# ChenKaiXuSan/Skiing_Analysis_PyTorch

Measured on AMD Instinct MI355X. Metric: 3D-pose frames/sec, 8-view 518px clips, higher is better.
Workload: dtype f16

## Files before the change

### include/skimi.h

```cpp
#ifndef SKIMI_H
#define SKIMI_H

#include <stddef.h>
#include <stdint.h>

#ifdef __cplusplus
extern "C" {
#endif

#define SKIMI_OK 0
#define SKIMI_ERR_ARG (-1)
#define SKIMI_ERR_HIP (-2)
#define SKIMI_ERR_STATE (-3)
#define SKIMI_ERR_WORKSPACE (-4)

#define SKIMI_F32 0
#define SKIMI_BF16 1
#define SKIMI_BF16X3_REC 2
#define SKIMI_FP8MX 3
#define SKIMI_F16 4

#define SKIMI_PREC_BF16 0
#define SKIMI_PREC_BF16X3 1
#define SKIMI_PREC_FP8 2
// ... 59 lines not shown
int skimi_gemm(const skimi_gemm_desc* d, void* stream);

#define SKIMI_GEMM_PATH_GENERIC 1
#define SKIMI_GEMM_PATH_SPLITK_ORDERED 2
#define SKIMI_GEMM_PATH_SPLITK_ATOMIC 3
#define SKIMI_GEMM_PATH_X3DMA_WIDE 4
#define SKIMI_GEMM_PATH_X3DMA_NARROW 5
#define SKIMI_GEMM_PATH_GEMM256 6
#define SKIMI_GEMM_PATH_CONV_WIN 7
int32_t skimi_gemm_last_path(void);

int skimi_quant_mx(const void* x, int32_t dtype, int64_t ldx, int64_t rows, int32_t K, void* payload, void* scales,
                   void* stream);
int skimi_layernorm_mx(const float* x, int64_t ldx, int64_t rows, int32_t C, const float* gamma, const float* beta,
                       float eps, void* payload, void* scales, void* stream);
int skimi_gemm_fp8(const void* A, const void* A_scales, const void* W, const void* W_scales, int32_t M, int32_t N,
                   int32_t K, const float* bias, int32_t act, const float* gamma, const float* resid, int64_t ldr,
                   void* out, int32_t out_dtype, int64_t ldo, void* out_scales, void* stream);

int skimi_conv3x3_n32_pack(const float* w, void* packed, int32_t C, void* stream);
int skimi_conv3x3_n32(const void* in_hi, const void* in_lo, const void* packed_w, const float* bias, float* out,
                      int32_t F, int32_t H, int32_t W, int32_t C, int32_t relu, void* stream);

int skimi_resample_u8(const uint8_t* in, uint8_t* out, int64_t outer, int32_t n_in, int32_t n_out, int64_t inner,
                      const int32_t* kk, const int32_t* bounds, int32_t ksize, void* stream);
int skimi_u8_hwc_to_f32_chw(const uint8_t* in, int32_t H, int32_t W, float* out, int32_t OH, int32_t OW, int32_t y_off,
                            int32_t x_off, float fill, void* stream);

int skimi_layernorm(const float* x, const float* x2, int64_t ldx, int64_t rows, int32_t C,
                    const float* gamma, const float* beta, float eps,
                    void* out, int32_t out_dtype, int64_t ldo, void* stream);

int skimi_qknorm_rope(void* qkv, int32_t dtype, int64_t tokens, int32_t heads,
                      const float* qn_w, const float* qn_b, const float* kn_w, const float* kn_b,
                      float eps, const int32_t* pos, const float* rope_cos, const float* rope_sin,
                      int32_t rope_npos, void* stream);

int skimi_attention(const void* qkv, void* out, int32_t dtype, int32_t batch, int32_t seq,
                    int32_t heads, int32_t head_dim, void* stream);
int skimi_attention_out(const void* qkv, void* out, int32_t dtype, int32_t out_dtype, int32_t batch, int32_t seq,
                        int32_t heads, int32_t head_dim, void* stream);

int skimi_qknorm_rope_scaled(void* qkv, int32_t dtype, int64_t tokens, int32_t heads,
                             const float* qn_w, const float* qn_b, const float* kn_w, const float* kn_b,
                             float eps, const int32_t* pos, const float* rope_cos, const float* rope_sin,
                             int32_t rope_npos, float q_scale, int32_t* q_scaled, void* stream);
// ... 80 lines not shown
```

### skiing_analysis_pytorch_amd/_lib.py

```python
from __future__ import annotations

import ctypes as C
from pathlib import Path

LIB_PATH = Path(__file__).resolve().parent / "lib" / "libskimi.so"

F32, BF16 = 0, 1
F16 = 4
BF16X3_REC = 2
FP8MX = 3
PREC_BF16, PREC_BF16X3, PREC_FP8 = 0, 1, 2
PREC_F16 = 3
ACT_NONE, ACT_RELU, ACT_GELU, ACT_SILU, ACT_SIGMOID = 0, 1, 2, 3, 4
GEMM_PATH_GENERIC, GEMM_PATH_SPLITK_ORDERED, GEMM_PATH_SPLITK_ATOMIC = 1, 2, 3
GEMM_PATH_X3DMA_WIDE, GEMM_PATH_X3DMA_NARROW, GEMM_PATH_GEMM256, GEMM_PATH_CONV_WIN = 4, 5, 6, 7


class SkimiError(RuntimeError):
    pass


class GemmDesc(C.Structure):

    _fields_ = [
# ... 29 lines not shown

_vp = C.c_void_p
_SIGNATURES = {
    "skimi_last_error": (C.c_char_p, []),
    "skimi_version": (C.c_int, []),
    "skimi_sizeof_gemm_desc": (C.c_int, []),
    "skimi_device_count": (C.c_int, []),
    "skimi_profile_start": (C.c_int, [C.c_int32, C.c_int64]),
    "skimi_profile_stop": (C.c_int, [C.POINTER(C.c_double), C.POINTER(C.c_int64), C.POINTER(C.c_double),
                                    C.POINTER(C.c_double)]),
    "skimi_gemm": (C.c_int, [C.POINTER(GemmDesc), _vp]),
    "skimi_gemm_last_path": (C.c_int32, []),
    "skimi_quant_mx": (C.c_int, [_vp, C.c_int32, C.c_int64, C.c_int64, C.c_int32, _vp, _vp, _vp]),
    "skimi_layernorm_mx": (C.c_int, [_vp, C.c_int64, C.c_int64, C.c_int32, _vp, _vp, C.c_float, _vp, _vp, _vp]),
    "skimi_gemm_fp8": (C.c_int, [_vp, _vp, _vp, _vp, C.c_int32, C.c_int32, C.c_int32, _vp, C.c_int32, _vp, _vp, C.c_int64,
                                 _vp, C.c_int32, C.c_int64, _vp, _vp]),
    "skimi_split_planes": (C.c_int, [_vp, C.c_int64, C.c_int64, C.c_int32, _vp, _vp, _vp]),
    "skimi_split_records": (C.c_int, [_vp, C.c_int64, C.c_int64, C.c_int32, _vp, _vp]),
    "skimi_resample_u8": (C.c_int, [_vp, _vp, C.c_int64, C.c_int32, C.c_int32, C.c_int64, _vp, _vp, C.c_int32, _vp]),
    "skimi_u8_hwc_to_f32_chw": (C.c_int, [_vp, C.c_int32, C.c_int32, _vp, C.c_int32, C.c_int32, C.c_int32, C.c_int32,
                                          C.c_float, _vp]),
    "skimi_conv3x3_n32_pack": (C.c_int, [_vp, _vp, C.c_int32, _vp]),
    "skimi_conv3x3_n32": (C.c_int, [_vp, _vp, _vp, _vp, _vp, C.c_int32, C.c_int32, C.c_int32, C.c_int32, C.c_int32, _vp]),
    "skimi_layernorm": (C.c_int, [_vp, _vp, C.c_int64, C.c_int64, C.c_int32, _vp, _vp, C.c_float, _vp,
                                  C.c_int32, C.c_int64, _vp]),
    "skimi_qknorm_rope": (C.c_int, [_vp, C.c_int32, C.c_int64, C.c_int32, _vp, _vp, _vp, _vp, C.c_float,
                                    _vp, _vp, _vp, C.c_int32, _vp]),
    "skimi_attention": (C.c_int, [_vp, _vp, C.c_int32, C.c_int32, C.c_int32, C.c_int32, C.c_int32, _vp]),
    "skimi_attention_out": (C.c_int, [_vp, _vp, C.c_int32, C.c_int32, C.c_int32, C.c_int32, C.c_int32, C.c_int32, _vp]),
    "skimi_qknorm_rope_scaled": (C.c_int, [_vp, C.c_int32, C.c_int64, C.c_int32, _vp, _vp, _vp, _vp, C.c_float,
                                           _vp, _vp, _vp, C.c_int32, C.c_float, C.POINTER(C.c_int32), _vp]),
    "skimi_attention_ex": (C.c_int, [_vp, _vp, C.c_int32, C.c_int32, C.c_int32, C.c_int32, C.c_int32, C.c_int32, C.c_int32,
                                     _vp, C.c_uint64, C.POINTER(C.c_int32), _vp]),
    "skimi_attention_x3_scratch_bytes": (C.c_uint64, [C.c_int64, C.c_int64]),
    "skimi_vp3d_create": (_vp, [C.c_int32, C.c_int32, C.c_int32, C.POINTER(C.c_int32), C.c_int32,
                                C.c_int32, C.c_int32]),
    "skimi_vp3d_destroy": (None, [_vp]),
    "skimi_vp3d_set_weight": (C.c_int, [_vp, C.c_char_p, _vp, C.c_int64]),
    "skimi_vp3d_finalize": (C.c_int, [_vp, C.c_int32]),
    "skimi_vp3d_receptive_field": (C.c_int32, [_vp]),
    "skimi_vp3d_workspace_bytes": (C.c_size_t, [_vp, C.c_int32, C.c_int32]),
    "skimi_vp3d_forward": (C.c_int, [_vp, _vp, _vp, C.c_int32, C.c_int32, _vp, C.c_size_t, _vp]),
    "skimi_pose_to_cameras": (C.c_int, [_vp, C.c_int64, C.c_int32, C.c_int32, _vp, _vp, _vp]),
    "skimi_unproject_depth": (C.c_int, [_vp, _vp, _vp, _vp, C.c_int32, C.c_int32, C.c_int32, _vp]),
    "skimi_triangulate_dlt": (C.c_int, [_vp, _vp, _vp, _vp, _vp, C.c_int64, C.c_int32, C.c_int32, _vp]),
    "skimi_icp_workspace_bytes": (C.c_size_t, [C.c_int64, C.c_int64]),
# ... 67 lines not shown
```

### skiing_analysis_pytorch_amd/csrc/api.hip

```cpp
#include <stdarg.h>

#include <mutex>
#include <vector>

#include "common.h"
#include "gemm_epilogue.h"
#include "kernels.h"

namespace skimi {

static thread_local char g_err[512] = "";

void set_error(const char* fmt, ...) {
    va_list ap;
    va_start(ap, fmt);
    vsnprintf(g_err, sizeof(g_err), fmt, ap);
    va_end(ap);
}

int lds_opt_in(std::atomic<unsigned>& done, const void* kernel, int bytes, const char* what) {
    int dev = 0;
    if (hipGetDevice(&dev) != hipSuccess) {
        set_error("hipGetDevice failed (%s)", what);
        return SKIMI_ERR_HIP;
    }
    const unsigned bit = 1u << (dev & 31);
    if (done.load(std::memory_order_acquire) & bit) return SKIMI_OK;
    const hipError_t e = hipFuncSetAttribute(kernel, hipFuncAttributeMaxDynamicSharedMemorySize, bytes);
    if (e != hipSuccess) {
        set_error("hipFuncSetAttribute(%s, %d bytes of LDS) failed: %s", what, bytes, hipGetErrorString(e));
// ... 96 lines not shown
}

int skimi_resample_u8(const uint8_t* in, uint8_t* out, int64_t outer, int32_t n_in, int32_t n_out, int64_t inner,
                      const int32_t* kk, const int32_t* bounds, int32_t ksize, void* stream) {
    return resample_u8_launch(in, out, outer, n_in, n_out, inner, kk, bounds, ksize, (hipStream_t)stream);
}

int skimi_u8_hwc_to_f32_chw(const uint8_t* in, int32_t H, int32_t W, float* out, int32_t OH, int32_t OW, int32_t y_off,
                            int32_t x_off, float fill, void* stream) {
    return u8_hwc_to_f32_chw_launch(in, H, W, out, OH, OW, y_off, x_off, fill, (hipStream_t)stream);
}

int skimi_conv3x3_n32_pack(const float* w, void* packed, int32_t C, void* stream) {
    SKIMI_CHECK_ARG(w && packed && C > 0, "skimi_conv3x3_n32_pack: bad arguments");
    return conv_direct_pack_launch(w, (unsigned short*)packed, C, (hipStream_t)stream);
}

int skimi_conv3x3_n32(const void* in_hi, const void* in_lo, const void* packed_w, const float* bias, float* out,
                      int32_t F, int32_t H, int32_t W, int32_t C, int32_t relu, void* stream) {
    return conv_direct_n32_launch((const unsigned short*)in_hi, (const unsigned short*)in_lo,
                                  (const unsigned short*)packed_w, bias, out, F, H, W, C, relu, (hipStream_t)stream);
}

int skimi_split_planes(const float* x, int64_t ld, int64_t rows, int32_t C, void* hi, void* lo, void* stream) {
    SKIMI_CHECK_ARG(x && hi && lo && rows > 0 && C > 0, "skimi_split_planes: bad arguments");
    return split_planes_launch(x, (long)ld, (long)rows, C, hi, lo, (hipStream_t)stream);
}

int skimi_split_records(const float* x, int64_t ld, int64_t rows, int32_t C, void* records, void* stream) {
    SKIMI_CHECK_ARG(x && records && rows > 0 && C > 0, "skimi_split_records: bad arguments");
    return split_records_launch(x, (long)ld, (long)rows, C, records, (hipStream_t)stream);
}

int skimi_quant_mx(const void* x, int32_t dtype, int64_t ldx, int64_t rows, int32_t K, void* payload, void* scales,
                   void* stream) {
    return quant_mx_launch(x, dtype, (long)ldx, (long)rows, K, payload, scales, (hipStream_t)stream);
}

int skimi_layernorm_mx(const float* x, int64_t ldx, int64_t rows, int32_t C, const float* gamma, const float* beta,
                       float eps, void* payload, void* scales, void* stream) {
    return layernorm_mx_launch(x, ldx, rows, C, gamma, beta, eps, payload, scales, (hipStream_t)stream);
}

int skimi_gemm_fp8(const void* A, const void* A_scales, const void* W, const void* W_scales, int32_t M, int32_t N,
                   int32_t K, const float* bias, int32_t act, const float* gamma, const float* resid, int64_t ldr,
                   void* out, int32_t out_dtype, int64_t ldo, void* out_scales, void* stream) {
// ... 70 lines not shown
```

### skiing_analysis_pytorch_amd/csrc/conv_direct.hip

```cpp
#include "common.h"
#include "kernels.h"

namespace skimi {

typedef __attribute__((address_space(3))) void lds_void;
typedef __attribute__((address_space(1))) const void gbl_void;

__device__ uint4 g_conv_zero_page[4] = {{0, 0, 0, 0}, {0, 0, 0, 0}, {0, 0, 0, 0}, {0, 0, 0, 0}};

constexpr int CD_WIN = 18 * 18;
constexpr int CD_IN_PLANE = 21 * 1024;
constexpr int CD_W_PLANE = 9 * 32 * 64;
constexpr int CD_BUF = 2 * CD_IN_PLANE + 2 * CD_W_PLANE;

__global__ void conv_direct_pack_kernel(const float* __restrict__ w, unsigned short* __restrict__ out, int Cin) {
    const long n = 32L * Cin * 9;
    for (long i = (long)blockIdx.x * 256 + threadIdx.x; i < n; i += (long)gridDim.x * 256) {
        const int c32 = (int)(i % 32);
        const int co = (int)((i / 32) % 32);
        const int tap = (int)((i / 1024) % 9);
        const int cs = (int)(i / 9216);
        const float v = w[((long)co * Cin + cs * 32 + c32) * 9 + tap];
        const unsigned short hi = f2bf(v);
        const unsigned short lo = f2bf(v - bf2f(hi));
// ... 157 lines not shown
}

int conv_direct_n32_launch(const unsigned short* in_hi, const unsigned short* in_lo, const unsigned short* w_packed,
                           const float* bias, float* out, int F, int H, int W, int C, int relu, hipStream_t st,
                           long px_stride) {
    SKIMI_CHECK_ARG(in_hi && in_lo && w_packed && out, "conv_direct: null buffer");
    SKIMI_CHECK_ARG(C % 32 == 0 && C >= 32 && F > 0 && H > 0 && W > 0, "conv_direct: bad shape");
    SKIMI_CHECK_ARG((((uintptr_t)in_hi | (uintptr_t)in_lo | (uintptr_t)w_packed) & 15) == 0, "conv_direct: 16-B alignment");
    constexpr size_t lds = 2ull * CD_BUF;
    SKIMI_LDS_OPT_IN(conv_direct_n32_kernel, lds, "conv_direct");
    ConvDirectArgs a;
    a.in_hi = in_hi; a.in_lo = in_lo; a.w = w_packed; a.bias = bias; a.out = out;
    a.F = F; a.H = H; a.W = W; a.C = C; a.relu = relu;
    a.px_stride = px_stride > 0 ? px_stride : C;
    a.tiles_x = (int)cdiv(W, 16);
    a.tiles_y = (int)cdiv(H, 16);
    const long nblk = (long)F * a.tiles_x * a.tiles_y;
    SKIMI_CHECK_ARG(nblk < (1l << 31), "conv_direct: grid too large");
    hipLaunchKernelGGL(conv_direct_n32_kernel, dim3((unsigned)nblk), dim3(512), lds, st, a);
    SKIMI_LAUNCH_CHECK();
    return SKIMI_OK;
}

}
```

### skiing_analysis_pytorch_amd/csrc/kernels.h

```cpp
#pragma once
#include "common.h"

namespace skimi {

int gemm_dispatch(const skimi_gemm_desc* d, hipStream_t st, void* scratch, size_t scratch_bytes,
                  int force_splitk);

int layernorm_launch(const float* x, const float* x2, int64_t ldx, int64_t rows, int C,
                     const float* gamma, const float* beta, float eps, void* out, int out_dtype,
                     int64_t ldo, hipStream_t st, int64_t grp_rows = 0, int64_t grp_stride = 0,
                     int64_t grp_off = 0);

int qknorm_rope_launch(void* qkv, int dtype, int64_t tokens, int heads, const float* qn_w,
                       const float* qn_b, const float* kn_w, const float* kn_b, float eps,
                       const int32_t* pos, const float* rope_cos, const float* rope_sin, int rope_npos,
                       hipStream_t st, float q_scale = 1.f, int* q_scaled = nullptr);

struct AttnArgs {
    const void* q;
    const void* k;
    const void* v;
    void* out;
    long q_row, k_row, v_row, o_row;
    long q_batch, k_batch, v_batch, o_batch;
    long q_head, k_head, v_head, o_head;
    int batch, heads, seq_q, seq_k, head_dim;
    float scale;
    int batch_inner = 0;
    long q_batch2 = 0, k_batch2 = 0, v_batch2 = 0, o_batch2 = 0;
    int q_prescaled = 0;
    int out_f16 = 0;
    void* out_mx = nullptr;
    void* out_mx_scales = nullptr;
    long mx_row = 0, mx_srow = 0;
};
bool attention_mx_output_ok(int dtype, int heads, int head_dim);
int attention_f32_launch(const AttnArgs& a, hipStream_t st);
int attention_bf16_launch(const AttnArgs& a, hipStream_t st);
int resample_u8_launch(const unsigned char* in, unsigned char* out, long outer, int n_in, int n_out, long inner,
                       const int* kk, const int* bounds, int ksize, hipStream_t st);
int u8_hwc_to_f32_chw_launch(const unsigned char* in, int H, int W, float* out, int OH, int OW, int y_off, int x_off,
                             float fill, hipStream_t st);
int conv_direct_pack_launch(const float* w, unsigned short* out, int Cin, hipStream_t st);
int conv_direct_n32_launch(const unsigned short* in_hi, const unsigned short* in_lo, const unsigned short* w_packed,
                           const float* bias, float* out, int F, int H, int W, int C, int relu, hipStream_t st,
                           long px_stride = 0);
void attention_q64_dispatch(const AttnArgs& a, hipStream_t st);
int attention_launch(const void* qkv, void* out, int dtype, int batch, int seq, int heads, int head_dim,
                     hipStream_t st, int q_prescaled = 0, void* x3_scratch = nullptr, size_t x3_scratch_bytes = 0,
                     int* out_records = nullptr,
                     int out_f16 = 0,
                     void* out_mx = nullptr, void* out_mx_scales = nullptr);
size_t attention_x3_scratch_bytes(long tokens, long row_elems);
int attention_x3_launch(const AttnArgs& a, long tokens, long row_elems, void* scratch, size_t scratch_bytes, hipStream_t st,
                        bool out_records = false);

int vp3d_im2col_launch(const float* x, float* a0, int B, int L, int Cin, int k, int Kpad, hipStream_t st);

int quant_mx_launch(const void* x, int dtype, long ldx, long rows, int K, void* q, void* scales, hipStream_t st);
int gemm_fp8_launch(const void* A, const void* As, const void* W, const void* Ws, int M, int N, int K, const float* bias, int act,
                    const float* gamma, const float* resid, long ldr, void* out, int out_dtype, long ldo, hipStream_t st,
                    void* out_scales = nullptr);
bool gemm_fp8_mx_output_ok(int M, int N);
int layernorm_mx_launch(const float* x, int64_t ldx, int64_t rows, int C, const float* gamma, const float* beta, float eps,
                        void* payload, void* scales, hipStream_t st);

int vp3d_expand_launch(const float* x, const float* w, int ldw, const float* bias, float* out_f32, void* out_rec, int B, int Lin,
                       int Cin, int taps, int C, hipStream_t st);
int vp3d_expand_mfma_launch(const float* x, const void* wfrag, int Kpad, const float* bias, float* out_f32, void* out_rec, int B,
// ... 7 lines not shown
```

### skiing_analysis_pytorch_amd/csrc/vggt.hip

```cpp
#include <math.h>
#include <string.h>

#include <map>
#include <memory>
#include <string>
#include <tuple>
#include <atomic>
#include <mutex>
#include <vector>

#include <stdlib.h>

#include "common.h"
#include "gemm_epilogue.h"
#include "kernels.h"
#include "track_kernels.h"
#include "vggt_kernels.h"

using namespace skimi;

namespace {

struct Lin {
    void* w = nullptr;
// ... 642 lines not shown
        if (!c.rc && !c.dry()) c.rc = bilinear_ac_launch(olow, o, adt, F, h0, w0, h1, w1, feat, c.st);
        prev = o;
        hh[r] = h1; ww[r] = w1;
    }
    const int h1 = hh[0], w1 = ww[0];
    const int f2 = w.feature_only ? feat : feat / 2;
    void* c1 = c.ar.alloc((size_t)F * h1 * w1 * f2 * es);
    if (prev_rec != nullptr) {
        auto d = c.desc(w.oc1.lin, prev_rec, SKIMI_BF16X3_REC, feat, F * h1 * w1, c1, adt, f2);
        c.conv_geom(d, w.oc1, F, h1, w1, h1, w1);
        d.x3_scratch = prev_rec + (size_t)F * h1 * w1 * feat * 4;
        d.x3_scratch_bytes = 256;
        if (!c.rc && !c.dry()) c.rc = gemm_dispatch(&d, c.st, c.slab, c.slab_bytes, 0);
    } else {
        auto d = c.desc(w.oc1.lin, prev, adt, feat, F * h1 * w1, c1, adt, f2);
        c.conv_geom(d, w.oc1, F, h1, w1, h1, w1);
        c.gemm(d);
    }
    const int Ho = ph * c.h->cfg.patch_size / w.down_ratio, Wo = pw * c.h->cfg.patch_size / w.down_ratio;
    const UvTab* uvt = w.pos_embed ? find_uv(c.tabs, Wo, Ho, f2) : nullptr;
    if (w.pos_embed && !uvt && !c.rc && !c.dry()) { set_error("uv table missing"); c.rc = SKIMI_ERR_STATE; }
    static const int no_direct = getenv("SKIMI_CONV_DIRECT") ? !atoi(getenv("SKIMI_CONV_DIRECT")) : 0;
    const bool direct = !w.feature_only && w.oc2a_direct != nullptr && adt == SKIMI_F32 && !no_direct;
    void* c2 = nullptr;
    if (direct) {
        const size_t pe = (size_t)F * Ho * Wo * f2;
        unsigned short* rec = (unsigned short*)c.ar.alloc(pe * 4);
        c2 = c.ar.alloc((size_t)F * Ho * Wo * 32 * es);
        if (!c.rc && !c.dry())
            c.rc = bilinear_ac_planes_launch((const float*)c1, rec, F, h1, w1, Ho, Wo, f2, c.st, uvt ? uvt->tx : nullptr,
                                             uvt ? uvt->ty : nullptr);
        if (!c.rc && !c.dry())
            c.rc = conv_direct_n32_launch(rec, rec + f2, w.oc2a_direct, w.oc2a.lin.b, (float*)c2, F, Ho, Wo, f2, 1, c.st,
                                          2L * f2);
    } else {
        const int udt = (w.feature_only && w.out_f32) ? SKIMI_F32 : adt;
        void* c1u = c.ar.alloc((size_t)F * Ho * Wo * f2 * Ctx::esz(udt));
        if (!c.rc && !c.dry())
            c.rc = dpt_fused_ln(w, f2, udt)
                       ? bilinear_ac_launch(c1, c1u, adt, F, h1, w1, Ho, Wo, f2, c.st, uvt ? uvt->tx : nullptr, uvt ? uvt->ty : nullptr, udt,
                                            w.out_ln->g, w.out_ln->b, 1e-5f)
                       : bilinear_ac_launch(c1, c1u, adt, F, h1, w1, Ho, Wo, f2, c.st, uvt ? uvt->tx : nullptr, uvt ? uvt->ty : nullptr, udt);
        if (w.feature_only) return c1u;
        c2 = c.ar.alloc((size_t)F * Ho * Wo * 32 * es);
        auto d = c.desc(w.oc2a.lin, c1u, adt, f2, F * Ho * Wo, c2, adt, 32);
        c.conv_geom(d, w.oc2a, F, Ho, Wo, Ho, Wo);
        d.act = SKIMI_ACT_RELU;
        c.gemm(d);
    }
    if (!c.rc && !c.dry())
        c.rc = dpt_out_launch(c2, adt, w.oc2b_w, w.oc2b_b, w.n_out, pts, conf, (long)F * Ho * Wo, act_mode, c.st);
    c.ar.release(mk);
    (void)H; (void)W;
    return nullptr;
// ... 509 lines not shown
```

### skiing_analysis_pytorch_amd/csrc/vggt_kernels.hip

```cpp
#include <algorithm>

#include "common.h"
#include "vggt_kernels.h"

namespace skimi {

static inline int grid_for(long n, int per_block = 256, int cap = 8192) {
    return (int)std::max<long>(1, std::min<long>(cdiv(n, per_block), cap));
}

template <typename T, bool F16 = false>
__global__ __launch_bounds__(256) void patch_gather_kernel(const float* __restrict__ img, T* __restrict__ out,
                                                           int F, int H, int W, int p, int Kp) {
    const int ph = H / p, pw = W / p, K = 3 * p * p;
    const long total = (long)F * ph * pw * Kp;
    const float mean[3] = {0.485f, 0.456f, 0.406f};
    const float stdv[3] = {0.229f, 0.224f, 0.225f};
    for (long i = (long)blockIdx.x * 256 + threadIdx.x; i < total; i += (long)gridDim.x * 256) {
        const int k = (int)(i % Kp);
        const long r = i / Kp;
        float v = 0.f;
        if (k < K) {
            const int px = (int)(r % pw);
            const int py = (int)((r / pw) % ph);
            const long f = r / ((long)pw * ph);
            const int c = k / (p * p);
// ... 129 lines not shown
    const int rowlen = W * C8;
    const float sy = H > 1 ? (float)(h - 1) / (float)(H - 1) : 0.f;
    const float sx = W > 1 ? (float)(w - 1) / (float)(W - 1) : 0.f;
    const int Y = (int)(blockIdx.y % (unsigned)H);
    const long n = blockIdx.y / (unsigned)H;
    for (int i = blockIdx.x * 256 + threadIdx.x; i < rowlen; i += gridDim.x * 256) {
        const int X = i / C8;
        const int c8 = i - X * C8;
        const float fy = sy * Y, fx = sx * X;
        const int y0 = min((int)fy, h - 1), x0 = min((int)fx, w - 1);
        const int y1 = min(y0 + 1, h - 1), x1 = min(x0 + 1, w - 1);
        const float ly1 = fminf(fmaxf(fy - y0, 0.f), 1.f), lx1 = fminf(fmaxf(fx - x0, 0.f), 1.f);
        const float ly0 = 1.f - ly1, lx0 = 1.f - lx1;
        const float* base = in + n * (long)h * w * C + c8 * 8;
        float p00[8], p01[8], p10[8], p11[8];
        auto ld8 = [&](const float* q, float* d) {
            const float4 a = *reinterpret_cast<const float4*>(q), b = *reinterpret_cast<const float4*>(q + 4);
            d[0] = a.x; d[1] = a.y; d[2] = a.z; d[3] = a.w; d[4] = b.x; d[5] = b.y; d[6] = b.z; d[7] = b.w;
        };
        ld8(base + ((long)y0 * w + x0) * C, p00);
        ld8(base + ((long)y0 * w + x1) * C, p01);
        ld8(base + ((long)y1 * w + x0) * C, p10);
        ld8(base + ((long)y1 * w + x1) * C, p11);
        float r[8];
#pragma unroll
        for (int k = 0; k < 8; ++k)
            r[k] = ly0 * (lx0 * p00[k] + lx1 * p01[k]) + ly1 * (lx0 * p10[k] + lx1 * p11[k]);
        if (tabx != nullptr) {
            const int half = C / 2, c = c8 * 8;
            float e[8];
            ld8(c < half ? tabx + (long)X * half + c : taby + (long)Y * half + (c - half), e);
#pragma unroll
            for (int k = 0; k < 8; ++k) r[k] += e[k];
        }
        bf16x8 hi, lo;
#pragma unroll
        for (int k = 0; k < 8; ++k) {
            const unsigned short hb = f2bf(r[k]);
            hi[k] = (short)hb;
            lo[k] = (short)f2bf(r[k] - bf2f(hb));
        }
        const long pix = ((n * H + Y) * (long)W + X) * 2 * C;
        if (slice_records) {
            const int c = c8 * 8;
            const long o = pix + (c >> 5) * 64 + (c & 31);
            __builtin_nontemporal_store(hi, reinterpret_cast<bf16x8*>(out + o));
            __builtin_nontemporal_store(lo, reinterpret_cast<bf16x8*>(out + o + 32));
        } else {
            const long o = pix + c8 * 8;
            __builtin_nontemporal_store(hi, reinterpret_cast<bf16x8*>(out + o));
            __builtin_nontemporal_store(lo, reinterpret_cast<bf16x8*>(out + o + C));
        }
    }
}

int bilinear_ac_planes_launch(const float* in, unsigned short* out, int N, int h, int w, int H, int W, int C, hipStream_t st,
                              const float* tabx, const float* taby, int slice_records, void* zpage) {
    SKIMI_CHECK_ARG(C % 16 == 0, "bilinear resize into planes needs C %% 16 == 0");
    SKIMI_CHECK_ARG(!slice_records || C % 32 == 0, "bilinear resize into records needs C %% 32 == 0");
    SKIMI_CHECK_ARG(tabx == nullptr || taby != nullptr, "fused uv pos embed needs both tables");
    SKIMI_CHECK_ARG((long)N * H < 65536, "bilinear resize into planes: N * H must be < 65536");
    const int rowlen = W * (C / 8);
    hipLaunchKernelGGL(bilinear_ac_planes_kernel, dim3((unsigned)cdiv(rowlen, 256), (unsigned)(N * H)), dim3(256), 0, st, in, out, N,
                       h, w, H, W, C, tabx, taby, slice_records, (uint4*)zpage);
// ... 117 lines not shown
template <typename T, int NOUT>
__global__ __launch_bounds__(256) void dpt_out_kernel(const T* __restrict__ in, const float* __restrict__ Wt,
                                                      const float* __restrict__ b, float* __restrict__ pts,
                                                      float* __restrict__ conf, long npix, int mode, bool f16 = false) {
    __shared__ float ws[NOUT * 32 + NOUT];
    for (int i = threadIdx.x; i < NOUT * 32 + NOUT; i += 256) ws[i] = i < NOUT * 32 ? Wt[i] : b[i - NOUT * 32];
    __syncthreads();
    for (long px = (long)blockIdx.x * 256 + threadIdx.x; px < npix; px += (long)gridDim.x * 256) {
        float v[32];
        if (sizeof(T) == 4) {
#pragma unroll
            for (int k = 0; k < 8; ++k) {
                const float4 t = *reinterpret_cast<const float4*>((const float*)in + px * 32 + 4 * k);
                v[4 * k] = t.x; v[4 * k + 1] = t.y; v[4 * k + 2] = t.z; v[4 * k + 3] = t.w;
            }
        } else {
#pragma unroll
            for (int k = 0; k < 4; ++k) {
                const bf16x8 t = *reinterpret_cast<const bf16x8*>((const unsigned short*)in + px * 32 + 8 * k);
#pragma unroll
                for (int j = 0; j < 8; ++j) v[8 * k + j] = x16tof((unsigned short)t[j], f16);
            }
        }
        float o[NOUT];
#pragma unroll
        for (int n = 0; n < NOUT; ++n) {
            float s = 0.f;
#pragma unroll
            for (int k = 0; k < 32; ++k) s += v[k] * ws[n * 32 + k];
            o[n] = s + ws[NOUT * 32 + n];
        }
#pragma unroll
        for (int n = 0; n < NOUT - 1; ++n) {
            float y = o[n];
            if (mode == 0) y = expf(y);
            else y = copysignf(expm1f(fabsf(y)), y) * (y != 0.f ? 1.f : 0.f);
            pts[px * (NOUT - 1) + n] = y;
        }
        conf[px] = 1.f + expf(o[NOUT - 1]);
    }
}

int dpt_out_launch(const void* in, int dtype, const float* W, const float* b, int n_out, float* pts, float* conf,
                   long npix, int mode, hipStream_t st) {
    SKIMI_CHECK_ARG(n_out == 2 || n_out == 4, "dpt output stage supports 2 or 4 channels (got %d)", n_out);
    dim3 g(grid_for(npix, 256, 16384)), blk(256);
#define GO(T, N) hipLaunchKernelGGL((dpt_out_kernel<T, N>), g, blk, 0, st, (const T*)in, W, b, pts, conf, npix, mode, dtype == SKIMI_F16)
    if (dtype == SKIMI_F32) { if (n_out == 2) GO(float, 2); else GO(float, 4); }
    else { if (n_out == 2) GO(unsigned short, 2); else GO(unsigned short, 4); }
#undef GO
    SKIMI_LAUNCH_CHECK();
    return SKIMI_OK;
}

__global__ void f32_to_bf16_kernel(const float* __restrict__ in, unsigned short* __restrict__ out, long n) {
    for (long i = (long)blockIdx.x * 256 + threadIdx.x; i < n; i += (long)gridDim.x * 256) out[i] = f2bf(in[i]);
}
int f32_to_bf16_launch(const float* in, void* out, long n, hipStream_t st) {
    hipLaunchKernelGGL(f32_to_bf16_kernel, dim3(grid_for(n)), dim3(256), 0, st, in, (unsigned short*)out, n);
    SKIMI_LAUNCH_CHECK();
    return SKIMI_OK;
}
// ... 80 lines not shown
```

### skiing_analysis_pytorch_amd/ops.py

```python
from __future__ import annotations

import ctypes as C
from typing import NamedTuple, Optional

import torch

from . import _lib
from ._lib import ACT_NONE, BF16, F16, F32, PREC_BF16, PREC_BF16X3, GemmDesc, check, lib, ptr


def _dt(t: torch.Tensor) -> int:
    if t.dtype == torch.float32:
        return F32
    if t.dtype == torch.bfloat16:
        return BF16
    if t.dtype == torch.float16:
        return F16
    raise TypeError(f"unsupported dtype {t.dtype}")


def _require_cuda(*ts):
    for t in ts:
        if t is not None and not t.is_cuda:
            raise _lib.SkimiError("libskimi ops need device (HBM) tensors; got a CPU tensor")
# ... 185 lines not shown
    assert out.numel() * out.element_size() >= need, "attention: `out` is too small"
    check(lib().skimi_attention_ex(ptr(qkv), ptr(out), _dt(qkv), odt, batch, seq, heads, head_dim, int(q_prescaled),
                                   ptr(x3_scratch), sc_bytes, C.byref(flag), _lib.current_stream()), "skimi_attention_ex")
    if mx:
        buf = out.view(torch.uint8).reshape(-1)
        return buf[:rows * Kp].view(rows, Kp), buf[rows * Kp:need].view(rows, Kp // 32)
    return (out, bool(flag.value)) if out_records else out


def conv3x3_n32(x, w, bias=None, relu=False):
    _require_cuda(x, w, bias)
    F_, H, W_, Cc = x.shape
    assert w.shape == (32, Cc, 3, 3) and Cc % 32 == 0
    planes = split_planes(x.reshape(-1, Cc).contiguous())
    packed = torch.empty(2 * 32 * Cc * 9, dtype=torch.bfloat16, device=x.device)
    st = _lib.current_stream()
    check(lib().skimi_conv3x3_n32_pack(ptr(w.contiguous()), ptr(packed), Cc, st), "skimi_conv3x3_n32_pack")
    out = torch.empty((F_, H, W_, 32), dtype=torch.float32, device=x.device)
    check(lib().skimi_conv3x3_n32(ptr(planes[0]), ptr(planes[1]), ptr(packed), ptr(bias), ptr(out), F_, H, W_, Cc,
                                  1 if relu else 0, st), "skimi_conv3x3_n32")
    return out


def split_records(x):
    _require_cuda(x)
    rows, Cc = x.shape
    out = torch.empty((rows, (Cc + 31) // 32, 2, 32), dtype=torch.bfloat16, device=x.device)
    check(lib().skimi_split_records(ptr(x), x.stride(0), rows, Cc, ptr(out), _lib.current_stream()), "skimi_split_records")
    return out


def records_buffer(rows, Cc, device="cuda"):
    return torch.empty(rows * ((Cc + 31) // 32) * 64 + 128, dtype=torch.bfloat16, device=device)


def x3_scratch_numel(rows, Cc):
    return rows * ((Cc + 31) // 32 * 32) + 64


def split_planes(x):
    _require_cuda(x)
    rows, Cc = x.shape
    out = torch.empty((2, rows, Cc), dtype=torch.bfloat16, device=x.device)
    check(lib().skimi_split_planes(ptr(x), x.stride(0), rows, Cc, ptr(out[0]), ptr(out[1]), _lib.current_stream()),
          "skimi_split_planes")
    return out
# ... 47 lines not shown
```

Before: 17.37.

## Fuse DPT head bilinear upsample, 3x3 conv and output projection into one kernel

Adds a conv_direct_up kernel that computes the bilinear upsample plus UV embedding on the fly into LDS as hi/lo bf16 planes. It then runs the 3x3 n32 conv with MFMA and applies ReLU and the 1x1 output head with exp/expm1 activations in the epilogue. It becomes the default path, so the upsampled record buffer and the intermediate c2 feature map are never written to or re-read from HBM. The trade-off is redundant bilinear gathers for the halo on every channel slice, extra register pressure from the gather buffers, and an alternate mode that fuses only the conv and head. The shared bilinear and output math is also factored into helpers.

```diff
diff --git a/include/skimi.h b/include/skimi.h
--- a/include/skimi.h
+++ b/include/skimi.h
@@ -105,6 +105,10 @@
 int skimi_conv3x3_n32(const void* in_hi, const void* in_lo, const void* packed_w, const float* bias, float* out,
                       int32_t F, int32_t H, int32_t W, int32_t C, int32_t relu, void* stream);
 
+int skimi_dpt_tail(const float* c1, int32_t F, int32_t h, int32_t w, int32_t H, int32_t W, int32_t C, const float* tabx,
+                   const float* taby, const void* packed_w, const float* bias, const float* w1, const float* b1, int32_t n_out,
+                   int32_t mode, float* pts, float* conf, int32_t path, void* scratch, void* stream);
+
 int skimi_resample_u8(const uint8_t* in, uint8_t* out, int64_t outer, int32_t n_in, int32_t n_out, int64_t inner,
                       const int32_t* kk, const int32_t* bounds, int32_t ksize, void* stream);
 int skimi_u8_hwc_to_f32_chw(const uint8_t* in, int32_t H, int32_t W, float* out, int32_t OH, int32_t OW, int32_t y_off,
diff --git a/skiing_analysis_pytorch_amd/_lib.py b/skiing_analysis_pytorch_amd/_lib.py
--- a/skiing_analysis_pytorch_amd/_lib.py
+++ b/skiing_analysis_pytorch_amd/_lib.py
@@ -75,6 +75,8 @@
                                           C.c_float, _vp]),
     "skimi_conv3x3_n32_pack": (C.c_int, [_vp, _vp, C.c_int32, _vp]),
     "skimi_conv3x3_n32": (C.c_int, [_vp, _vp, _vp, _vp, _vp, C.c_int32, C.c_int32, C.c_int32, C.c_int32, C.c_int32, _vp]),
+    "skimi_dpt_tail": (C.c_int, [_vp, C.c_int32, C.c_int32, C.c_int32, C.c_int32, C.c_int32, C.c_int32, _vp, _vp, _vp, _vp,
+                                 _vp, _vp, C.c_int32, C.c_int32, _vp, _vp, C.c_int32, _vp, _vp]),
     "skimi_layernorm": (C.c_int, [_vp, _vp, C.c_int64, C.c_int64, C.c_int32, _vp, _vp, C.c_float, _vp,
                                   C.c_int32, C.c_int64, _vp]),
     "skimi_qknorm_rope": (C.c_int, [_vp, C.c_int32, C.c_int64, C.c_int32, _vp, _vp, _vp, _vp, C.c_float,
diff --git a/skiing_analysis_pytorch_amd/csrc/api.hip b/skiing_analysis_pytorch_amd/csrc/api.hip
--- a/skiing_analysis_pytorch_amd/csrc/api.hip
+++ b/skiing_analysis_pytorch_amd/csrc/api.hip
@@ -6,6 +6,7 @@
 #include "common.h"
 #include "gemm_epilogue.h"
 #include "kernels.h"
+#include "vggt_kernels.h"
 
 namespace skimi {
 
@@ -148,6 +149,24 @@
                                   (const unsigned short*)packed_w, bias, out, F, H, W, C, relu, (hipStream_t)stream);
 }
 
+int skimi_dpt_tail(const float* c1, int32_t F, int32_t h, int32_t w, int32_t H, int32_t W, int32_t C, const float* tabx,
+                   const float* taby, const void* packed_w, const float* bias, const float* w1, const float* b1, int32_t n_out,
+                   int32_t mode, float* pts, float* conf, int32_t path, void* scratch, void* stream) {
+    SKIMI_CHECK_ARG(c1 && packed_w && pts && conf && path >= 0 && path <= 2, "skimi_dpt_tail: bad arguments");
+    SKIMI_CHECK_ARG(path == 1 || scratch != nullptr, "skimi_dpt_tail: paths 0 and 2 need scratch");
+    const hipStream_t st = (hipStream_t)stream;
+    const unsigned short* wp = (const unsigned short*)packed_w;
+    if (path == 1) return conv_direct_up_launch(c1, h, w, tabx, taby, nullptr, wp, bias, w1, b1, n_out, mode, pts, conf, F, H, W, C, st);
+    unsigned short* rec = (unsigned short*)scratch;
+    int rc = bilinear_ac_planes_launch(c1, rec, F, h, w, H, W, C, st, tabx, taby);
+    if (rc) return rc;
+    if (path == 2) return conv_direct_up_launch(nullptr, 0, 0, nullptr, nullptr, rec, wp, bias, w1, b1, n_out, mode, pts, conf, F, H, W, C, st);
+    float* c2 = (float*)(rec + (size_t)F * H * W * 2 * C);
+    rc = conv_direct_n32_launch(rec, rec + C, wp, bias, c2, F, H, W, C, 1, st, 2L * C);
+    if (rc) return rc;
+    return dpt_out_launch(c2, SKIMI_F32, w1, b1, n_out, pts, conf, (long)F * H * W, mode, st);
+}
+
 int skimi_split_planes(const float* x, int64_t ld, int64_t rows, int32_t C, void* hi, void* lo, void* stream) {
     SKIMI_CHECK_ARG(x && hi && lo && rows > 0 && C > 0, "skimi_split_planes: bad arguments");
     return split_planes_launch(x, (long)ld, (long)rows, C, hi, lo, (hipStream_t)stream);
diff --git a/skiing_analysis_pytorch_amd/csrc/conv_direct.hip b/skiing_analysis_pytorch_amd/csrc/conv_direct.hip
--- a/skiing_analysis_pytorch_amd/csrc/conv_direct.hip
+++ b/skiing_analysis_pytorch_amd/csrc/conv_direct.hip
@@ -1,4 +1,5 @@
 #include "common.h"
+#include "dpt_tail.h"
 #include "kernels.h"
 
 namespace skimi {
@@ -203,4 +204,272 @@
     return SKIMI_OK;
 }
 
-}
+constexpr int CU_TASKS = 3;
+constexpr int CU_EP_PITCH = 36;
+
+struct ConvUpArgs {
+    const float* c1;
+    const float* tabx;
+    const float* taby;
+    const unsigned short* rec;
+    const unsigned short* w;
+    const float* bias;
+    const float* w2;
+    const float* b2;
+    float* pts;
+    float* conf;
+    int F, hs, ws, H, W, C, mode, tiles_x, tiles_y;
+};
+
+template <bool UP, int NOUT>
+__global__ __launch_bounds__(512) void conv_direct_up_kernel(const ConvUpArgs p) {
+    extern __shared__ __attribute__((aligned(16))) char smem[];
+    const int tid = threadIdx.x, lane = tid & 63;
+    const int wave = __builtin_amdgcn_readfirstlane(tid >> 6);
+    const int l31 = lane & 31, lh = lane >> 5;
+
+    int bid = blockIdx.x;
+    const int tx = bid % p.tiles_x;
+    bid /= p.tiles_x;
+    const int ty = bid % p.tiles_y;
+    const int f = bid / p.tiles_y;
+    const int y0 = ty * 16, x0 = tx * 16;
+    const int nsl = p.C / 32;
+    const unsigned short* zero = reinterpret_cast<const unsigned short*>(g_conv_zero_page);
+
+    int w_off[3], w_piece[3];
+    int nw = 0;
+#pragma unroll
+    for (int j = 0; j < 3; ++j) {
+        const int q = wave + 8 * j;
+        w_piece[j] = q;
+        w_off[j] = 0;
+        if (q < 18) {
+            nw = j + 1;
+            const int row = 16 * q + (lane >> 2);
+            const int sc = (lane & 3) ^ ((row >> 2) & 3);
+            w_off[j] = row * 32 + sc * 8;
+        }
+    }
+    auto stage_w = [&](int buf, int s) {
+        char* base = smem + buf * CD_BUF;
+        const unsigned short* ws = p.w + (long)s * 2 * 9216;
+#pragma unroll
+        for (int j = 0; j < 3; ++j) {
+            if (j < nw) {
+                char* dst = base + 2 * CD_IN_PLANE + w_piece[j] * 1024;
+                __builtin_amdgcn_global_load_lds((gbl_void*)(ws + w_off[j]), (lds_void*)dst, 16, 0, 0);
+                __builtin_amdgcn_global_load_lds((gbl_void*)(ws + 9216 + w_off[j]), (lds_void*)(dst + CD_W_PLANE), 16, 0, 0);
+            }
+        }
+    };
+
+    const float* src = p.c1 + (long)f * p.hs * p.ws * p.C;
+    const float sy = p.H > 1 ? (float)(p.hs - 1) / (float)(p.H - 1) : 0.f;
+    const float sx = p.W > 1 ? (float)(p.ws - 1) / (float)(p.W - 1) : 0.f;
+    struct Task {
+        int Y, X, lds;
+        bool in;
+        int y0, x0, y1, x1;
+        float fy, fx;
+    };
+    auto task = [&](int j) {
+        Task k;
+        const int t = tid + 512 * j;
+        const int px = t >> 2, c = t & 3;
+        const int hy = px / 18, hx = px - hy * 18;
+        const int Y = y0 - 1 + hy, X = x0 - 1 + hx;
+        k.lds = t < 4 * CD_WIN ? px * 64 + ((c ^ (((hx + 2 * hy) >> 2) & 3)) << 4) : -1;
+        k.in = t < 4 * CD_WIN && Y >= 0 && Y < p.H && X >= 0 && X < p.W;
+        k.Y = min(max(Y, 0), p.H - 1);
+        k.X = min(max(X, 0), p.W - 1);
+        k.fy = sy * k.Y;
+        k.fx = sx * k.X;
+        k.y0 = min((int)k.fy, p.hs - 1);
+        k.x0 = min((int)k.fx, p.ws - 1);
+        k.y1 = min(k.y0 + 1, p.hs - 1);
+        k.x1 = min(k.x0 + 1, p.ws - 1);
+        return k;
+    };
+    float P[CU_TASKS][4][8], E[CU_TASKS][8];
+    auto ld8 = [](const float* q, float* d) {
+        const float4 a = *reinterpret_cast<const float4*>(q), b = *reinterpret_cast<const float4*>(q + 4);
+        d[0] = a.x; d[1] = a.y; d[2] = a.z; d[3] = a.w; d[4] = b.x; d[5] = b.y; d[6] = b.z; d[7] = b.w;
+    };
+    const bool uv = p.tabx != nullptr;
+    auto gather = [&](int s) {
+        const int half = p.C / 2, ch = s * 32 + (tid & 3) * 8;
+        const float* q = src + ch;
+#pragma unroll
+        for (int j = 0; j < CU_TASKS; ++j) {
+            const Task k = task(j);
+            ld8(q + (k.y0 * p.ws + k.x0) * p.C, P[j][0]);
+            ld8(q + (k.y0 * p.ws + k.x1) * p.C, P[j][1]);
+            ld8(q + (k.y1 * p.ws + k.x0) * p.C, P[j][2]);
+            ld8(q + (k.y1 * p.ws + k.x1) * p.C, P[j][3]);
+            ld8(!uv ? q : ch < half ? p.tabx + k.X * half + ch : p.taby + k.Y * half + (ch - half), E[j]);
+        }
+    };
+    auto commit = [&](int buf) {
+        char* base = smem + buf * CD_BUF;
+#pragma unroll
+        for (int j = 0; j < CU_TASKS; ++j) {
+            const Task k = task(j);
+            const float ly1 = fminf(fmaxf(k.fy - k.y0, 0.f), 1.f), lx1 = fminf(fmaxf(k.fx - k.x0, 0.f), 1.f);
+            const float ly0 = 1.f - ly1, lx0 = 1.f - lx1;
+            bf16x8 hi, lo;
+            bilinear_split8(P[j][0], P[j][1], P[j][2], P[j][3], uv ? E[j] : nullptr, lx0, lx1, ly0, ly1, hi, lo);
+            const bf16x8 z = {0, 0, 0, 0, 0, 0, 0, 0};
+            if (k.lds >= 0) {
+                *reinterpret_cast<bf16x8*>(base + k.lds) = k.in ? hi : z;
+                *reinterpret_cast<bf16x8*>(base + CD_IN_PLANE + k.lds) = k.in ? lo : z;
+            }
+        }
+    };
+
+    long in_off[3];
+    int nin = 0;
+    if constexpr (!UP) {
+#pragma unroll
+        for (int j = 0; j < 3; ++j) {
+            const int q = wave + 8 * j;
+            in_off[j] = -1;
+            if (q < 21) {
+                nin = j + 1;
+                const int px = 16 * q + (lane >> 2);
+                const int hy = px / 18, hx = px - hy * 18;
+                const int y = y0 - 1 + hy, x = x0 - 1 + hx;
+                const int sc = (lane & 3) ^ (((hx + 2 * hy) >> 2) & 3);
+                if (px < CD_WIN && y >= 0 && y < p.H && x >= 0 && x < p.W)
+                    in_off[j] = (((long)f * p.H + y) * p.W + x) * 2 * p.C + sc * 8;
+            }
+        }
+    }
+    auto stage_rec = [&](int buf, int s) {
+        char* base = smem + buf * CD_BUF;
+#pragma unroll
+        for (int j = 0; j < 3; ++j) {
+            if (j < nin) {
+                const bool ok = in_off[j] >= 0;
+                const unsigned short* sh = ok ? p.rec + in_off[j] + s * 32 : zero;
+                const unsigned short* sl = ok ? p.rec + in_off[j] + p.C + s * 32 : zero;
+                char* dst = base + (wave + 8 * j) * 1024;
+                __builtin_amdgcn_global_load_lds((gbl_void*)sh, (lds_void*)dst, 16, 0, 0);
+                __builtin_amdgcn_global_load_lds((gbl_void*)sl, (lds_void*)(dst + CD_IN_PLANE), 16, 0, 0);
+            }
+        }
+    };
+
+    const int col = ((l31 & 15) + ((l31 >> 4) ? 14 : 0)) & 15;
+    int a_off[9][2];
+#pragma unroll
+    for (int tap = 0; tap < 9; ++tap) {
+        const int dy = tap / 3, dx = tap - dy * 3;
+        const int hy = 2 * wave + (l31 >> 4) + dy, hx = col + dx;
+        const int px = hy * 18 + hx;
+#pragma unroll
+        for (int ks = 0; ks < 2; ++ks) a_off[tap][ks] = px * 64 + (((2 * ks + lh) ^ (((hx + 2 * hy) >> 2) & 3)) << 4);
+    }
+    int b_off[2];
+#pragma unroll
+    for (int ks = 0; ks < 2; ++ks) b_off[ks] = l31 * 64 + (((2 * ks + lh) ^ ((l31 >> 2) & 3)) << 4);
+
+    f32x16 acc;
+#pragma unroll
+    for (int r = 0; r < 16; ++r) acc[r] = 0.f;
+
+    if constexpr (UP) {
+        gather(0);
+        stage_w(0, 0);
+        commit(0);
+    } else {
+        stage_rec(0, 0);
+        stage_w(0, 0);
+    }
+    __syncthreads();
+    for (int s = 0; s < nsl; ++s) {
+        const int cur = s & 1;
+        const bool next = s + 1 < nsl;
+        if (next) {
+            if constexpr (UP) gather(s + 1);
+            else stage_rec(cur ^ 1, s + 1);
+            stage_w(cur ^ 1, s + 1);
+        }
+        const char* ih = smem + cur * CD_BUF;
+        const char* wh = ih + 2 * CD_IN_PLANE;
+#pragma unroll
+        for (int tap = 0; tap < 9; ++tap) {
+#pragma unroll
+            for (int ks = 0; ks < 2; ++ks) {
+                const bf16x8 a_hi = *reinterpret_cast<const bf16x8*>(ih + a_off[tap][ks]);
+                const bf16x8 a_lo = *reinterpret_cast<const bf16x8*>(ih + CD_IN_PLANE + a_off[tap][ks]);
+                const bf16x8 w_hi = *reinterpret_cast<const bf16x8*>(wh + tap * 2048 + b_off[ks]);
+                const bf16x8 w_lo = *reinterpret_cast<const bf16x8*>(wh + CD_W_PLANE + tap * 2048 + b_off[ks]);
+                acc = __builtin_amdgcn_mfma_f32_32x32x16_bf16(a_lo, w_hi, acc, 0, 0, 0);
+                acc = __builtin_amdgcn_mfma_f32_32x32x16_bf16(a_hi, w_lo, acc, 0, 0, 0);
+                acc = __builtin_amdgcn_mfma_f32_32x32x16_bf16(a_hi, w_hi, acc, 0, 0, 0);
+            }
+        }
+        if constexpr (UP) {
+            if (next) commit(cur ^ 1);
+        }
+        __syncthreads();
+    }
+
+    float* ep = reinterpret_cast<float*>(smem) + wave * 32 * CU_EP_PITCH;
+    const float bs = p.bias ? p.bias[l31] : 0.f;
+#pragma unroll
+    for (int r = 0; r < 16; ++r) {
+        const int pix = (r & 3) + 8 * (r >> 2) + 4 * lh;
+        ep[pix * CU_EP_PITCH + l31] = fmaxf(acc[r] + bs, 0.f);
+    }
+    __syncthreads();
+    const int y = y0 + 2 * wave + (l31 >> 4), x = x0 + col;
+    if (lh == 0 && y < p.H && x < p.W) {
+        float v[32];
+#pragma unroll
+        for (int k = 0; k < 32; k += 4) {
+            const float4 t = *reinterpret_cast<const float4*>(ep + l31 * CU_EP_PITCH + k);
+            v[k] = t.x; v[k + 1] = t.y; v[k + 2] = t.z; v[k + 3] = t.w;
+        }
+        const long px = ((long)f * p.H + y) * p.W + x;
+        dpt_out_pixel<NOUT>(v, p.w2, p.b2, p.mode, p.pts + px * (NOUT - 1), p.conf + px);
+    }
+}
+
+int conv_direct_up_launch(const float* c1, int h, int w, const float* tabx, const float* taby, const unsigned short* rec,
+                          const unsigned short* w_packed, const float* bias, const float* w2, const float* b2, int n_out,
+                          int mode, float* pts, float* conf, int F, int H, int W, int C, hipStream_t st) {
+    SKIMI_CHECK_ARG((c1 != nullptr) != (rec != nullptr), "conv_direct_up: exactly one of c1 / records");
+    SKIMI_CHECK_ARG(w_packed && w2 && b2 && pts && conf, "conv_direct_up: null buffer");
+    SKIMI_CHECK_ARG(n_out == 2 || n_out == 4, "conv_direct_up: 2 or 4 output channels (got %d)", n_out);
+    SKIMI_CHECK_ARG(C % 32 == 0 && C >= 32 && F > 0 && H > 0 && W > 0, "conv_direct_up: bad shape");
+    SKIMI_CHECK_ARG(!c1 || (h > 0 && w > 0 && (long)h * w * C < (1l << 31)), "conv_direct_up: bad source map");
+    SKIMI_CHECK_ARG((tabx == nullptr) == (taby == nullptr), "conv_direct_up: UV embedding needs both tables");
+    SKIMI_CHECK_ARG(!c1 || (long)W * (C / 2) < (1l << 31) && (long)H * (C / 2) < (1l << 31), "conv_direct_up: UV tables too large");
+    SKIMI_CHECK_ARG((((uintptr_t)c1 | (uintptr_t)tabx | (uintptr_t)taby | (uintptr_t)rec | (uintptr_t)w_packed) & 15) == 0,
+                    "conv_direct_up: 16-B alignment");
+    constexpr size_t lds = 2ull * CD_BUF;
+    static_assert(8 * 32 * CU_EP_PITCH * 4 <= lds, "epilogue tile");
+    static_assert(512 * CU_TASKS >= 4 * CD_WIN, "window tasks");
+    ConvUpArgs a;
+    a.c1 = c1; a.tabx = tabx; a.taby = taby; a.rec = rec; a.w = w_packed; a.bias = bias; a.w2 = w2; a.b2 = b2;
+    a.pts = pts; a.conf = conf;
+    a.F = F; a.hs = h; a.ws = w; a.H = H; a.W = W; a.C = C; a.mode = mode;
+    a.tiles_x = (int)cdiv(W, 16);
+    a.tiles_y = (int)cdiv(H, 16);
+    const long nblk = (long)F * a.tiles_x * a.tiles_y;
+    SKIMI_CHECK_ARG(nblk < (1l << 31), "conv_direct_up: grid too large");
+#define GO(UP_, N_)                                                                                   \
+    do {                                                                                              \
+        SKIMI_LDS_OPT_IN((conv_direct_up_kernel<UP_, N_>), lds, "conv_direct_up");                    \
+        hipLaunchKernelGGL((conv_direct_up_kernel<UP_, N_>), dim3((unsigned)nblk), dim3(512), lds, st, a); \
+    } while (0)
+    if (c1) { if (n_out == 2) GO(true, 2); else GO(true, 4); }
+    else { if (n_out == 2) GO(false, 2); else GO(false, 4); }
+#undef GO
+    SKIMI_LAUNCH_CHECK();
+    return SKIMI_OK;
+}
+
+}
diff --git a/skiing_analysis_pytorch_amd/csrc/dpt_tail.h b/skiing_analysis_pytorch_amd/csrc/dpt_tail.h
--- /dev/null
+++ b/skiing_analysis_pytorch_amd/csrc/dpt_tail.h
@@ -0,0 +1,44 @@
+#pragma once
+#include "common.h"
+
+namespace skimi {
+
+__device__ __forceinline__ void bilinear_split8(const float* p00, const float* p01, const float* p10, const float* p11,
+                                                const float* e, float lx0, float lx1, float ly0, float ly1,
+                                                bf16x8& hi, bf16x8& lo) {
+#pragma clang fp contract(off)
+#pragma unroll
+    for (int k = 0; k < 8; ++k) {
+        const float t0 = lx0 * p00[k] + lx1 * p01[k];
+        const float t1 = lx0 * p10[k] + lx1 * p11[k];
+        float r = ly0 * t0 + ly1 * t1;
+        if (e != nullptr) r += e[k];
+        const unsigned short hb = f2bf(r);
+        hi[k] = (short)hb;
+        lo[k] = (short)f2bf(r - bf2f(hb));
+    }
+}
+
+template <int NOUT>
+__device__ __forceinline__ void dpt_out_pixel(const float* v, const float* wt, const float* b, int mode, float* pts,
+                                              float* conf) {
+#pragma clang fp contract(off)
+    float o[NOUT];
+#pragma unroll
+    for (int n = 0; n < NOUT; ++n) {
+        float s = 0.f;
+#pragma unroll
+        for (int k = 0; k < 32; ++k) s += v[k] * wt[n * 32 + k];
+        o[n] = s + b[n];
+    }
+#pragma unroll
+    for (int n = 0; n < NOUT - 1; ++n) {
+        float y = o[n];
+        if (mode == 0) y = expf(y);
+        else y = copysignf(expm1f(fabsf(y)), y) * (y != 0.f ? 1.f : 0.f);
+        pts[n] = y;
+    }
+    *conf = 1.f + expf(o[NOUT - 1]);
+}
+
+}
diff --git a/skiing_analysis_pytorch_amd/csrc/kernels.h b/skiing_analysis_pytorch_amd/csrc/kernels.h
--- a/skiing_analysis_pytorch_amd/csrc/kernels.h
+++ b/skiing_analysis_pytorch_amd/csrc/kernels.h
@@ -45,6 +45,9 @@
 int conv_direct_n32_launch(const unsigned short* in_hi, const unsigned short* in_lo, const unsigned short* w_packed,
                            const float* bias, float* out, int F, int H, int W, int C, int relu, hipStream_t st,
                            long px_stride = 0);
+int conv_direct_up_launch(const float* c1, int h, int w, const float* tabx, const float* taby, const unsigned short* rec,
+                          const unsigned short* w_packed, const float* bias, const float* w2, const float* b2, int n_out,
+                          int mode, float* pts, float* conf, int F, int H, int W, int C, hipStream_t st);
 void attention_q64_dispatch(const AttnArgs& a, hipStream_t st);
 int attention_launch(const void* qkv, void* out, int dtype, int batch, int seq, int heads, int head_dim,
                      hipStream_t st, int q_prescaled = 0, void* x3_scratch = nullptr, size_t x3_scratch_bytes = 0,
diff --git a/skiing_analysis_pytorch_amd/csrc/vggt.hip b/skiing_analysis_pytorch_amd/csrc/vggt.hip
--- a/skiing_analysis_pytorch_amd/csrc/vggt.hip
+++ b/skiing_analysis_pytorch_amd/csrc/vggt.hip
@@ -688,14 +688,30 @@
     if (w.pos_embed && !uvt && !c.rc && !c.dry()) { set_error("uv table missing"); c.rc = SKIMI_ERR_STATE; }
     static const int no_direct = getenv("SKIMI_CONV_DIRECT") ? !atoi(getenv("SKIMI_CONV_DIRECT")) : 0;
     const bool direct = !w.feature_only && w.oc2a_direct != nullptr && adt == SKIMI_F32 && !no_direct;
+    static const int up_mode = getenv("SKIMI_CONV_DIRECT_UP") ? atoi(getenv("SKIMI_CONV_DIRECT_UP")) : 1;
     void* c2 = nullptr;
+    if (direct && up_mode == 1) {
+        if (!c.rc && !c.dry())
+            c.rc = conv_direct_up_launch((const float*)c1, h1, w1, uvt ? uvt->tx : nullptr, uvt ? uvt->ty : nullptr, nullptr,
+                                         w.oc2a_direct, w.oc2a.lin.b, w.oc2b_w, w.oc2b_b, w.n_out, act_mode, pts, conf, F, Ho,
+                                         Wo, f2, c.st);
+        c.ar.release(mk);
+        return nullptr;
+    }
     if (direct) {
         const size_t pe = (size_t)F * Ho * Wo * f2;
         unsigned short* rec = (unsigned short*)c.ar.alloc(pe * 4);
-        c2 = c.ar.alloc((size_t)F * Ho * Wo * 32 * es);
         if (!c.rc && !c.dry())
             c.rc = bilinear_ac_planes_launch((const float*)c1, rec, F, h1, w1, Ho, Wo, f2, c.st, uvt ? uvt->tx : nullptr,
                                              uvt ? uvt->ty : nullptr);
+        if (up_mode == 2) {
+            if (!c.rc && !c.dry())
+                c.rc = conv_direct_up_launch(nullptr, 0, 0, nullptr, nullptr, rec, w.oc2a_direct, w.oc2a.lin.b, w.oc2b_w,
+                                             w.oc2b_b, w.n_out, act_mode, pts, conf, F, Ho, Wo, f2, c.st);
+            c.ar.release(mk);
+            return nullptr;
+        }
+        c2 = c.ar.alloc((size_t)F * Ho * Wo * 32 * es);
         if (!c.rc && !c.dry())
             c.rc = conv_direct_n32_launch(rec, rec + f2, w.oc2a_direct, w.oc2a.lin.b, (float*)c2, F, Ho, Wo, f2, 1, c.st,
                                           2L * f2);
diff --git a/skiing_analysis_pytorch_amd/csrc/vggt_kernels.hip b/skiing_analysis_pytorch_amd/csrc/vggt_kernels.hip
--- a/skiing_analysis_pytorch_amd/csrc/vggt_kernels.hip
+++ b/skiing_analysis_pytorch_amd/csrc/vggt_kernels.hip
@@ -2,6 +2,7 @@
 
 #include "common.h"
 #include "vggt_kernels.h"
+#include "dpt_tail.h"
 
 namespace skimi {
 
@@ -177,24 +178,13 @@
         ld8(base + ((long)y0 * w + x1) * C, p01);
         ld8(base + ((long)y1 * w + x0) * C, p10);
         ld8(base + ((long)y1 * w + x1) * C, p11);
-        float r[8];
-#pragma unroll
-        for (int k = 0; k < 8; ++k)
-            r[k] = ly0 * (lx0 * p00[k] + lx1 * p01[k]) + ly1 * (lx0 * p10[k] + lx1 * p11[k]);
+        float e[8];
         if (tabx != nullptr) {
             const int half = C / 2, c = c8 * 8;
-            float e[8];
             ld8(c < half ? tabx + (long)X * half + c : taby + (long)Y * half + (c - half), e);
-#pragma unroll
-            for (int k = 0; k < 8; ++k) r[k] += e[k];
         }
         bf16x8 hi, lo;
-#pragma unroll
-        for (int k = 0; k < 8; ++k) {
-            const unsigned short hb = f2bf(r[k]);
-            hi[k] = (short)hb;
-            lo[k] = (short)f2bf(r[k] - bf2f(hb));
-        }
+        bilinear_split8(p00, p01, p10, p11, tabx != nullptr ? e : nullptr, lx0, lx1, ly0, ly1, hi, lo);
         const long pix = ((n * H + Y) * (long)W + X) * 2 * C;
         if (slice_records) {
             const int c = c8 * 8;
@@ -358,22 +348,7 @@
                 for (int j = 0; j < 8; ++j) v[8 * k + j] = x16tof((unsigned short)t[j], f16);
             }
         }
-        float o[NOUT];
-#pragma unroll
-        for (int n = 0; n < NOUT; ++n) {
-            float s = 0.f;
-#pragma unroll
-            for (int k = 0; k < 32; ++k) s += v[k] * ws[n * 32 + k];
-            o[n] = s + ws[NOUT * 32 + n];
-        }
-#pragma unroll
-        for (int n = 0; n < NOUT - 1; ++n) {
-            float y = o[n];
-            if (mode == 0) y = expf(y);
-            else y = copysignf(expm1f(fabsf(y)), y) * (y != 0.f ? 1.f : 0.f);
-            pts[px * (NOUT - 1) + n] = y;
-        }
-        conf[px] = 1.f + expf(o[NOUT - 1]);
+        dpt_out_pixel<NOUT>(v, ws, ws + NOUT * 32, mode, pts + px * (NOUT - 1), conf + px);
     }
 }
 
diff --git a/skiing_analysis_pytorch_amd/ops.py b/skiing_analysis_pytorch_amd/ops.py
--- a/skiing_analysis_pytorch_amd/ops.py
+++ b/skiing_analysis_pytorch_amd/ops.py
@@ -231,6 +231,24 @@
     return out
 
 
+def dpt_tail(c1, H, W_, w3, b3, w1, b1, mode, tabx=None, taby=None, path=1):
+    _require_cuda(c1, w3, b3, w1, b1, tabx, taby)
+    c1, w1 = c1.contiguous(), w1.contiguous()
+    F_, h, w_, Cc = c1.shape
+    n_out = w1.shape[0]
+    assert w3.shape == (32, Cc, 3, 3) and w1.shape == (n_out, 32) and Cc % 32 == 0
+    st = _lib.current_stream()
+    packed = torch.empty(2 * 32 * Cc * 9, dtype=torch.bfloat16, device=c1.device)
+    check(lib().skimi_conv3x3_n32_pack(ptr(w3.contiguous()), ptr(packed), Cc, st), "skimi_conv3x3_n32_pack")
+    pts = torch.empty((F_, H, W_, n_out - 1), dtype=torch.float32, device=c1.device)
+    conf = torch.empty((F_, H, W_), dtype=torch.float32, device=c1.device)
+    scratch = None if path == 1 else torch.empty(F_ * H * W_ * (4 * Cc + 128), dtype=torch.uint8, device=c1.device)
+    check(lib().skimi_dpt_tail(ptr(c1), F_, h, w_, H, W_, Cc, ptr(tabx), ptr(taby), ptr(packed), ptr(b3),
+                               ptr(w1), ptr(b1), n_out, mode, ptr(pts), ptr(conf), path, ptr(scratch), st),
+          "skimi_dpt_tail")
+    return pts, conf
+
+
 def split_records(x):
     _require_cuda(x)
     rows, Cc = x.shape
```

Result: no change. 17.50, median of 6 (+0.7%).
